# SamiPerttu/fundsp

Hardware: AMD Instinct MI355X
Metric: Msamples/s (whole node) for 65536-voice SVF+FM graph (higher is better)
Workload: dtype f32

## Files before the change

fundsp_amd/csrc/fd_device.hpp:

```cpp
#pragma once

#include "fd_nodes.hpp"
#include "fd_plan.hpp"
#include "fd_seq.hpp"

namespace fd {

constexpr int TILE_STRIDE = 68;

struct VLoad {
    const float* p;
    size_t stride;
    int slot;
    FD_D void f(float& x, FieldKind, const char*) { x = p[(size_t)slot++ * stride]; }
    FD_D void fi(float& x, FieldKind, const char*, int) { x = p[(size_t)slot++ * stride]; }
    FD_D void u32(uint32_t& x, FieldKind, const char*) { x = f2u(p[(size_t)slot++ * stride]); }
    FD_D void u64(uint64_t& x, FieldKind, const char*) {
        uint32_t lo = f2u(p[(size_t)slot * stride]);
        uint32_t hi = f2u(p[(size_t)(slot + 1) * stride]);
        slot += 2;
        x = ((uint64_t)hi << 32) | lo;
    }
    FD_D void enter(int) {}
    FD_D void leave() {}
// ... 2368 lines not shown
            }
        }
    }
    auto rounds_of = [&](auto* tag) {
        using GG = typename Pointee<decltype(tag)>::type;
        using T0 = Seg<GG, 0, 1>;
        using T1 = Seg<GG, 1, 2>;
        using T2 = Seg<GG, 2, 3>;
        GG& gg = reinterpret_cast<GG&>(g);
        auto loop = [&](auto&& block) {
            for (size_t it = 0; it < rounds; it++) {
                if (run && it >= (size_t)stage && it - stage < nblocks)
                    block(it - stage);
                __syncthreads();
            }
        };
        if (stage == 0) loop([&](size_t j) { ts_stage<T0, GG, true, W>(gg, R::cut[0][part], R::cut[0][part + 1], lane, nullptr, hand[grp][0][j & 1]); });
        else if (stage == 1) loop([&](size_t j) { ts_stage<T1, GG, false, W>(gg, R::cut[1][part], R::cut[1][part + 1], lane, hand[grp][0][j & 1], hand[grp][1][j & 1]); });
        else loop([&](size_t j) { pipe_stage<T2, GG, MODE_PROCESS, StageCfg<64, W, false, true, 64, OLM, FD_PIPE_PREFETCH != 0, MCM, (GPW == 2)>>(gg, 0, j * 64, 64, 64, T, V, lane, outw, nullptr, hand[grp][1][j & 1], nullptr, &mxl); });
    };
    using GL = typename LpOf<G>::type;
    bool lp = false;
    if constexpr (!SameType<GL, G>::v && FD_LP_ENABLE)
        lp = __builtin_amdgcn_ballot_w64(run && !lp_ok(g)) == 0ull && __builtin_amdgcn_ballot_w64(run) != 0ull;
    if (stage == 2) __builtin_amdgcn_s_setprio(1);
    if (lp) rounds_of((GL*)nullptr); else rounds_of((G*)nullptr);
    if (live && active && part == 0) {
        VStore<false> st{slots + v, stride, 0};
        VGate::W<VStore<false>> gate{&st, true};
        if (stage == 0) S0::visit(g, gate); else if (stage == 1) S1::visit(g, gate); else S2::visit(g, gate);
    }
}

template <class G, int GPW>
__global__ __launch_bounds__(64 * Ts3Roles<GPW>::WAVES) void k_render_ts3(float* __restrict__ slots, size_t stride, size_t V,
                                                                          float* __restrict__ out, size_t T, const void* aux) {
    if constexpr (TsPlan<G>::ok) render_ts3_body<G, GPW>(slots, stride, V, out, T, aux);
}
template <class G, int GPW, int MIX>
__global__ __launch_bounds__(64 * Ts3Roles<GPW>::WAVES) void k_render_ts3_mix(float* __restrict__ slots, size_t stride, size_t V,
                                                                              float* __restrict__ part, size_t T, const void* aux,
                                                                              const float* __restrict__ panw) {
    if constexpr (TsPlan<G>::ok) render_ts3_body<G, GPW, MIX>(slots, stride, V, part, T, aux, panw);
}

constexpr int PFS = 65;
template <class G>
struct PlanarPlan {
    static constexpr PipePlan P2 = pipe_plan<G>(2);
    static constexpr int N = Chain<G>::N;
    template <int S, int K1> struct Tiles {
        using S0 = Seg<G, 0, S == 1 ? N : K1>;
        using S1 = Seg<G, S == 1 ? 0 : K1, N>;
        static constexpr int W = S >= 2 ? S0::OUT : 0;
        static constexpr bool LATE_GIN = S >= 2 && S1::USES_GIN;
        static constexpr int D = G::IN > 0 ? (LATE_GIN ? S + 1 : 2) : 0;
        static constexpr int UNITS = G::IN * D + 2 * W * (S - 1) + 2 * G::OUT;
        static constexpr int SUB = UNITS <= 4 ? 32 : UNITS <= 9 ? 16 : UNITS <= 18 ? 8 : 0;
        static constexpr int WAVES = S + 1 + (G::IN > 0 ? 1 : 0);
        static constexpr bool ok = SUB >= 8 && WAVES <= 4 && G::OUT > 0;
    };
    static constexpr bool two_ok() {
        if constexpr (P2.S == 2) return Tiles<2, P2.K1>::ok; else return false;
    }
    static constexpr bool two = two_ok();
    static constexpr int S = two ? 2 : (Tiles<1, N>::ok ? 1 : 0);
    static constexpr int K1 = two ? P2.K1 : N;
    using T = Tiles<(S >= 1 ? S : 1), K1>;
};

template <class G, int MODE, int S, int K1, int GPW = 4>
FD_D void render_pipe_planar_body(float* __restrict__ slots, size_t stride, size_t V, const float* __restrict__ in,
                                  float* __restrict__ out, size_t T, size_t fstride, const void* aux, float* ring, uint32_t ring_cap) {
    using TL = typename PlanarPlan<G>::template Tiles<S, K1>;
    constexpr int NI = G::IN, NO = G::OUT;
    constexpr bool FEED = NI > 0;
// ... 154 lines not shown
        while (n > 0) { buf[k++] = (char)('0' + n % 10); n /= 10; }
        while (k > 0) put(buf[--k]);
    }
    FD_D void prefix() {
        for (int i = 0; i < depth; i++) { if (i) put('.'); putn(path[i]); }
        put(':');
    }
    FD_D void line(const char* name, int index, const char* suffix, int kind) {
        prefix();
        puts_(name);
        if (index >= 0) { put('['); putn(index); put(']'); }
        puts_(suffix);
        put(' ');
        putn(kind);
        put('\n');
    }
    FD_D void f(float&, FieldKind k, const char* name) { line(name, -1, "", (int)k); }
    FD_D void fi(float&, FieldKind k, const char* name, int index) { line(name, index, "", (int)k); }
    FD_D void u32(uint32_t&, FieldKind k, const char* name) { line(name, -1, "", (int)k); }
    FD_D void u64(uint64_t&, FieldKind k, const char* name) { line(name, -1, ".lo", (int)k); line(name, -1, ".hi", (int)k); }
    FD_D void enter(int i) { if (depth < 32) path[depth] = i; depth++; }
    FD_D void leave() { depth--; }
    bool keeps = false;
    FD_D void stale() { keeps = true; }
};
template <class G>
struct JitPipeSmall {
    static constexpr PipePlan P = pipe_plan<G>(0);
    static constexpr bool on = P.S >= 1 && Cost<G>::v >= 150;
    template <int GPW> static constexpr int threads() { return on ? 16 * GPW * PipeGeom<G::IN, (P.S >= 1 ? P.S : 1)>::WAVES : 64; }
};
template <class G, int GPW>
FD_D void jit_ts3_body(float* __restrict__ slots, size_t stride, size_t V, float* __restrict__ out, size_t T, const void* aux) {
    if constexpr (TsPlan<G>::ok) render_ts3_body<G, GPW>(slots, stride, V, out, T, aux);
}
template <class G, int GPW, int MIX>
FD_D void jit_ts3_mix_body(float* __restrict__ slots, size_t stride, size_t V, float* __restrict__ part, size_t T, const void* aux, const float* __restrict__ panw) {
    if constexpr (TsPlan<G>::ok && (MIX == MIX_SUM ? G::OUT <= 2 : G::OUT == 1)) render_ts3_body<G, GPW, MIX>(slots, stride, V, part, T, aux, panw);
}

template <class G, int MODE>
FD_D void jit_pipe_body(float* __restrict__ slots, size_t stride, size_t V, const float* __restrict__ in,
                        float* __restrict__ out, size_t T, const void* aux, float* ring, uint32_t ring_cap) {
    constexpr PipePlan P = pipe_plan<G>(0);
    if constexpr (P.S >= 1) render_pipe_body<G, MODE, P.S, P.K1, P.K2>(slots, stride, V, in, out, T, aux, ring, ring_cap);
}
template <class G, int MODE, int GPW>
FD_D void jit_pipe_small_body(float* __restrict__ slots, size_t stride, size_t V, const float* __restrict__ in,
                              float* __restrict__ out, size_t T, const void* aux, float* ring, uint32_t ring_cap) {
    constexpr PipePlan P = pipe_plan<G>(0);
    if constexpr (JitPipeSmall<G>::on) render_pipe_body<G, MODE, P.S, P.K1, P.K2, GPW>(slots, stride, V, in, out, T, aux, ring, ring_cap);
}
template <class G, int MODE, int MIX>
FD_D void jit_pipe_mix_body(float* __restrict__ slots, size_t stride, size_t V, const float* __restrict__ in,
                            float* __restrict__ part, size_t T, const void* aux, float* ring, uint32_t ring_cap, const float* __restrict__ panw) {
    constexpr PipePlan P = pipe_plan<G>(0);
    if constexpr (P.S >= 1 && (MIX == MIX_SUM || G::OUT == 1)) {
        if constexpr (MixGeom<(MIX == MIX_PAN ? 1 : G::OUT), 4, PipeTiles<G, P.S, P.K1, P.K2, 4>::SUB>::ok)
            render_pipe_body<G, MODE, P.S, P.K1, P.K2, 4, MIX>(slots, stride, V, in, part, T, aux, ring, ring_cap, panw);
    }
}
constexpr bool jit_mix_channels_ok(int channels) { return (31 * 1024) / 4 / (channels * MIX_ROW * 4) >= 8; }
static_assert(jit_mix_channels_ok(3) && !jit_mix_channels_ok(4) && MixGeom<3, 4, 64>::ok && !MixGeom<4, 4, 64>::ok, "fused mix-down: at most three output channels at four voice groups per workgroup");
template <class G, int MODE>
FD_D void jit_events_mix_body(float* __restrict__ slots, size_t stride, size_t V, const float* __restrict__ in, float* __restrict__ part, size_t T,
                              const double* __restrict__ ev, const int* __restrict__ fade, double time0, double sr, const void* aux, float* ring,
                              uint32_t ring_cap) {
    if constexpr (G::OUT <= 2) render_events_body<G, MODE, true>(slots, stride, V, in, part, T, ev, fade, time0, sr, aux, ring, ring_cap);
}
template <class G, int MODE>
FD_D void jit_score_mix_body(float* __restrict__ slots, size_t stride, size_t V, const float* __restrict__ in, float* __restrict__ part, size_t T,
// ... 10 lines not shown
FD_D void jit_pipe_planar_body(float* __restrict__ slots, size_t stride, size_t V, const float* __restrict__ in,
                               float* __restrict__ out, size_t T, size_t fstride, const void* aux, float* ring, uint32_t ring_cap) {
    using PP = PlanarPlan<G>;
    if constexpr (PP::S >= 1) render_pipe_planar_body<G, MODE, PP::S, PP::K1>(slots, stride, V, in, out, T, fstride, aux, ring, ring_cap);
}
template <class G>
struct JitPipePlanarThreads {
    static constexpr int v = PlanarPlan<G>::S >= 1 ? 256 * PlanarPlan<G>::T::WAVES : 64;
};
template <class G>
struct JitPipeThreads {
    static constexpr PipePlan P = pipe_plan<G>(0);
    static constexpr int v = P.S >= 1 ? 64 * PipeGeom<G::IN, (P.S >= 1 ? P.S : 1)>::WAVES : 64;
};

template <class G>
constexpr GraphTraits graph_traits(bool run_time) {
    constexpr PipePlan P = pipe_plan<G>(0);
    constexpr bool heavy = Cost<G>::v >= 150, ts = TsPlan<G>::ok;
    GraphTraits t{};
    t.nin = G::IN, t.nout = G::OUT, t.nrings = G::RINGS;
    t.wpb_planar = RenderGeom<G, LAYOUT_PLANAR>::WPB;
    for (int want = 0; want < 4; want++) t.pipe_stages[want] = !run_time ? pipe_plan<G>(want).S : (want == 1 && pipe_plan<G>(1).S < 1) ? 0 : P.S;
    t.pipe_min_t = PipeMinT<G>::v;
    t.pipe_threads = P.S >= 1 ? JitPipeThreads<G>::v : 0;
    t.pipe_planar_threads = PlanarPlan<G>::S >= 1 ? JitPipePlanarThreads<G>::v : 0;
    t.planar_stages = PlanarPlan<G>::S;
    t.wide_waves = run_time && WideChain<G>::on ? WideChain<G>::W : 0;
    t.heavy = heavy;
    t.small_groups_planar = t.small_groups_mix = heavy && !run_time;
    t.ts_ok = ts, t.ts_round2 = ts && !run_time, t.ts_mix_ok = ts && (!run_time || G::OUT <= 2);
    t.mix_sum_ok = !run_time || jit_mix_channels_ok(G::OUT);
    t.has_fast = !SameType<typename FastOf<G>::type, G>::v;
    return t;
}
template <class G>
FD_D void describe_body(char* out, int cap, GraphTraits* traits) {
    if (threadIdx.x != 0 || blockIdx.x != 0) return;
    G g;
    VDescribeDev d{out, 0, cap, {0}, 0};
    g.visit(d);
    out[d.pos] = 0;
    GraphTraits t = graph_traits<G>(true);
    t.note_fresh = G::RINGS == 0 && !d.keeps;
    *traits = t;
}

}
```

fundsp_amd/csrc/fd_engine.hpp:

```cpp
#pragma once

#include <functional>
#include <string>
#include <type_traits>
#include <vector>

#include "fd_device.hpp"
#include "fd_opts.hpp"

namespace fd {

struct SlotInfo {
    std::string name;
    int kind;
};

struct VDescribe {
    std::vector<SlotInfo>* out;
    std::vector<int> path;
    std::string prefix() const {
        std::string s;
        for (size_t i = 0; i < path.size(); i++) {
            if (i) s += ".";
            s += std::to_string(path[i]);
// ... 68 lines not shown
struct RenderArgs {
    float* slots; size_t stride, V; const float* in; float* out; size_t T, fstride; const void* aux; float* ring; uint32_t ring_cap;
    const float* panw;
    hipStream_t s;
};
template <int N> using IntC = std::integral_constant<int, N>;
template <class G, class F>
void with_gpw(int gpw, F&& f) {
    if constexpr (Cost<G>::v >= 150) {
        if (gpw == 1) return f(IntC<1>{});
        if (gpw == 2) return f(IntC<2>{});
    }
    f(IntC<4>{});
}
template <class G, int MODE, int WANT, int MIX = MIX_NONE>
void launch_pipe(const RenderPlan& p, const RenderArgs& a) {
    constexpr PipePlan P = pipe_plan<G>(WANT);
    if constexpr (P.S >= 1) {
        constexpr int WAVES = PipeGeom<G::IN, P.S>::WAVES;
        with_gpw<G>(p.gpw, [&](auto gpw) {
            constexpr int GPW = decltype(gpw)::value;
            if constexpr (MIX == MIX_NONE)
                hipLaunchKernelGGL((k_render_pipe<G, MODE, P.S, P.K1, P.K2, GPW>), dim3(p.grid), dim3(16 * GPW * WAVES), 0, a.s, a.slots, a.stride, a.V,
                                   a.in, a.out, a.T, a.aux, a.ring, a.ring_cap);
            else
                hipLaunchKernelGGL((k_render_pipe_mix<G, MODE, P.S, P.K1, P.K2, GPW, MIX>), dim3(p.grid), dim3(16 * GPW * WAVES), 0, a.s, a.slots,
                                   a.stride, a.V, a.in, a.out, a.T, a.aux, a.ring, a.ring_cap, a.panw);
        });
    }
}
template <class G, int MIX>
void launch_ts(const RenderPlan& p, const RenderArgs& a) {
    auto ts3 = [&](auto gpw) {
        constexpr int GPW = decltype(gpw)::value, THREADS = 64 * Ts3Roles<GPW>::WAVES;
        if constexpr (MIX != MIX_NONE)
            hipLaunchKernelGGL((k_render_ts3_mix<G, GPW, MIX>), dim3(p.grid), dim3(THREADS), 0, a.s, a.slots, a.stride, a.V, a.out, a.T, a.aux, a.panw);
        else
            hipLaunchKernelGGL((k_render_ts3<G, GPW>), dim3(p.grid), dim3(THREADS), 0, a.s, a.slots, a.stride, a.V, a.out, a.T, a.aux);
    };
    if constexpr (MIX == MIX_NONE)
        if (p.ts_round2) {
            if (p.ts_round2 == 2) hipLaunchKernelGGL((k_render_ts<G, 2, 2>), dim3(p.grid), dim3(64 * 5), 0, a.s, a.slots, a.stride, a.V, a.out, a.T, a.aux);
            else hipLaunchKernelGGL((k_render_ts<G, 2, 1>), dim3(p.grid), dim3(64 * 4), 0, a.s, a.slots, a.stride, a.V, a.out, a.T, a.aux);
            return;
        }
    if (p.gpw == 1) ts3(IntC<1>{});
    else ts3(IntC<2>{});
}
template <class G> struct TspKernel { static constexpr bool ok = false; };
template <class G> void launch_tsp(const RenderPlan& p, const RenderArgs& a);
template <class G, int MODE, int LAYOUT>
void launch_single(const RenderPlan& p, const RenderArgs& a) {
    constexpr int WPB = RenderGeom<G, LAYOUT>::WPB;
    const size_t fstride = LAYOUT == LAYOUT_VOICE_MINOR ? (size_t)p.vpw : a.fstride;
    hipLaunchKernelGGL((k_render<G, MODE, LAYOUT, WPB>), dim3(p.grid), dim3(64 * WPB), 0, a.s, a.slots, a.stride, a.V, a.in, a.out, a.T, fstride, a.aux,
                       a.ring, a.ring_cap);
}
template <class G, int MODE>
void launch_render_mode(const RenderPlan& p, const RenderArgs& a, int layout) {
    if (p.family == LK_PIPELINE_PLANAR) {
        using PP = PlanarPlan<G>;
        if constexpr (PP::S >= 1)
            with_gpw<G>(p.gpw, [&](auto gpw) {
                constexpr int GPW = decltype(gpw)::value;
                hipLaunchKernelGGL((k_render_pipe_planar<G, MODE, PP::S, PP::K1, GPW>), dim3(p.grid), dim3(64 * GPW * PP::T::WAVES), 0, a.s, a.slots,
                                   a.stride, a.V, a.in, a.out, a.T, a.fstride, a.aux, a.ring, a.ring_cap);
            });
// ... 179 lines not shown
```

fundsp_amd/csrc/fd_jit.hip:

```cpp
#ifndef _GNU_SOURCE
#define _GNU_SOURCE 1
#endif
#include <dlfcn.h>
#include <link.h>
#include <limits.h>
#include <stdlib.h>
#include <hip/hiprtc.h>

#include <cstring>
#include <fstream>
#include <map>
#include <memory>
#include <mutex>
#include <cstdio>
#include <sstream>

#include "fd_engine.hpp"
#include "fd_resynth.hpp"

namespace fd {

int jit_compile_src(const std::string& src, const std::string& type_expr, std::vector<char>* code, std::string* log);
std::string jit_source_mix(const std::string& type_expr, const std::string& prelude);
std::string jit_source_score(const std::string& type_expr, const std::string& prelude);
// ... 253 lines not shown
        std::string log;
        const std::string type = which ? "typename fd::FastOf<" + jm->type_expr + ">::type" : jm->type_expr;
        if (jit_compile_src(jit_source_mix(type, jm->prelude), jm->type_expr, &mm->code, &log) == 0) jm->mix[which] = mm;
        else {
            jm->mix_failed[which] = true;
            fprintf(stderr, "fundsp_hip: the mix-down / time-split kernels of this graph failed to compile: %s\n", log.c_str());
        }
    }
    return jm->mix[which].get();
}

void jit_render(JitModule* jm, float* slots, size_t stride, size_t V, const float* in, float* outp, size_t T, size_t fstride,
                int layout, int mode, const void* aux, float* ring, uint32_t ring_cap, hipStream_t s, JitModule* base, int which) {
    if (V == 0 || T == 0) return;
    const JitFuncs* f = jm->get();
    if (!f) return jit_launch_failed();
    GraphTraits traits = jm->traits;
    const size_t cus = (size_t)simd_count() / 4;
    const bool aligned = (((uintptr_t)in | (uintptr_t)outp) & 15) == 0;
    RenderPlan p = plan_render(traits, tl_opts, cus, V, T, layout, mode, fstride, aligned);
    const JitMix::Dev* tf = nullptr;
    if (p.family == LK_TIME_SPLIT) {
        JitMix* mm = jit_extra_module(base, which);
        tf = mm ? mm->get() : nullptr;
        if (!tf) {
            traits.ts_ok = false;
            p = plan_render(traits, tl_opts, cus, V, T, layout, mode, fstride, aligned);
        }
    }
    tl_opts.last_kernel = p.family;
    const unsigned gpw = (unsigned)p.gpw;
    if (p.family == LK_TIME_SPLIT) {
        void* targs[] = {&slots, &stride, &V, &outp, &T, &aux};
        hipModuleLaunchKernel(tf->ts[gpw - 1], p.grid, 1, 1, 64u * (gpw == 1 ? Ts3Roles<1>::WAVES : Ts3Roles<2>::WAVES), 1, 1, 0, s, targs, nullptr);
        return;
    }
    if (p.family == LK_PIPELINE) {
        void* pargs[] = {&slots, &stride, &V, &in, &outp, &T, &aux, &ring, &ring_cap};
        hipModuleLaunchKernel(gpw == 4 ? f->pipe[mode] : f->pipe_small[gpw - 1][mode], p.grid, 1, 1, (unsigned)traits.pipe_threads / 4 * gpw, 1, 1, 0, s, pargs,
                              nullptr);
        return;
    }
    if (p.family == LK_SINGLE_WAVE && layout == LAYOUT_VOICE_MINOR) fstride = (size_t)p.vpw;
    void* args[] = {&slots, &stride, &V, &in, &outp, &T, &fstride, &aux, &ring, &ring_cap};
    if (p.family == LK_WIDE_CHAIN)
        hipModuleLaunchKernel(f->wide[mode][layout], p.grid, 1, 1, 64u * (unsigned)traits.wide_waves, 1, 1, 0, s, args, nullptr);
    else if (p.family == LK_PIPELINE_PLANAR)
        hipModuleLaunchKernel(f->pipe_planar[mode], p.grid, 1, 1, (unsigned)traits.pipe_planar_threads, 1, 1, 0, s, args, nullptr);
    else
        hipModuleLaunchKernel(f->render[mode][layout], p.grid, 1, 1, 64 * gpw, 1, 1, 0, s, args, nullptr);
}

}

std::string jit_source(const std::string& type_expr, const std::string& prelude) {
    std::string s;
    s += "#include \"fd_device.hpp\"\n";
    if (!prelude.empty()) s += "namespace fd {\n" + prelude + "\n}\n";
    s += "namespace fd { using JitG = " + type_expr + "; }\n";
    s += "using fd::JitG;\n";
    s += "constexpr int JIT_WPB0 = fd::RenderGeom<JitG, 0>::WPB;\nconstexpr int JIT_WPB1 = fd::RenderGeom<JitG, 1>::WPB;\n";
    s += "extern \"C\" __global__ __launch_bounds__(64) void jit_lifecycle(float* slots, size_t stride, size_t first, "
         "size_t count, int op, double sr, const uint64_t* seeds, const void* aux, float* ring, uint32_t cap) {\n"
         "  fd::lifecycle_body<JitG>(slots, stride, first, count, op, sr, seeds, aux, ring, cap); }\n";
    for (int mode = 0; mode < 2; mode++)
        for (int layout = 0; layout < 2; layout++) {
            std::string m = std::to_string(mode), l = std::to_string(layout);
// ... 32 lines not shown
        s += "extern \"C\" __global__ __launch_bounds__(JIT_PIPE_PLANAR_THREADS) void jit_pipe_planar_" + m +
             "(float* __restrict__ slots, size_t stride, size_t V, const float* __restrict__ in, float* __restrict__ out, "
             "size_t T, size_t fstride, const void* aux, float* ring, uint32_t cap) {\n"
             "  fd::jit_pipe_planar_body<JitG, " + m + ">(slots, stride, V, in, out, T, fstride, aux, ring, cap); }\n";
    }
    for (int mode = 0; mode < 2; mode++) {
        std::string m = std::to_string(mode);
        s += "extern \"C\" __global__ __launch_bounds__(256) void jit_events_" + m +
             "(float* __restrict__ slots, size_t stride, size_t V, const float* __restrict__ in, float* __restrict__ out, "
             "size_t T, const double* __restrict__ ev, const int* __restrict__ fade, double time0, double sr, const void* aux, "
             "float* ring, uint32_t cap) {\n"
             "  fd::render_events_body<JitG, " + m + ">(slots, stride, V, in, out, T, ev, fade, time0, sr, aux, ring, cap); }\n";
    }
    s += "extern \"C\" __global__ void jit_describe(char* out, int cap, fd::GraphTraits* traits) { fd::describe_body<JitG>(out, cap, traits); }\n";
    return s;
}

std::string jit_source_mix(const std::string& type_expr, const std::string& prelude) {
    std::string s;
    s += "#include \"fd_device.hpp\"\n";
    if (!prelude.empty()) s += "namespace fd {\n" + prelude + "\n}\n";
    s += "namespace fd { using JitG = " + type_expr + "; }\nusing fd::JitG;\n";
    s += "constexpr int JIT_PIPE_THREADS = fd::JitPipeThreads<JitG>::v;\n";
    for (int mix = 1; mix <= 2; mix++)
        for (int mode = 0; mode < 2; mode++) {
            std::string m = std::to_string(mode), x = std::to_string(mix);
            s += "extern \"C\" __global__ __launch_bounds__(JIT_PIPE_THREADS) void jit_pipe_mix_" + x + "_" + m +
                 "(float* __restrict__ slots, size_t stride, size_t V, const float* __restrict__ in, float* __restrict__ part, "
                 "size_t T, const void* aux, float* ring, uint32_t cap, const float* __restrict__ panw) {\n"
                 "  fd::jit_pipe_mix_body<JitG, " + m + ", " + x + ">(slots, stride, V, in, part, T, aux, ring, cap, panw); }\n";
        }
    for (int g = 1; g <= 2; g++) {
        std::string gs = std::to_string(g);
        s += "extern \"C\" __global__ __launch_bounds__(64 * fd::Ts3Roles<" + gs + ">::WAVES) void jit_ts3_g" + gs +
             "(float* __restrict__ slots, size_t stride, size_t V, float* __restrict__ out, size_t T, const void* aux) {\n"
             "  fd::jit_ts3_body<JitG, " + gs + ">(slots, stride, V, out, T, aux); }\n";
        for (int mix = 1; mix <= 2; mix++) {
            std::string x = std::to_string(mix);
            s += "extern \"C\" __global__ __launch_bounds__(64 * fd::Ts3Roles<" + gs + ">::WAVES) void jit_ts3_mix_g" + gs + "_" + x +
                 "(float* __restrict__ slots, size_t stride, size_t V, float* __restrict__ part, size_t T, const void* aux, const float* __restrict__ panw) {\n"
                 "  fd::jit_ts3_mix_body<JitG, " + gs + ", " + x + ">(slots, stride, V, part, T, aux, panw); }\n";
        }
    }
    for (int mode = 0; mode < 2; mode++) {
        std::string m = std::to_string(mode);
        s += "extern \"C\" __global__ __launch_bounds__(256) void jit_events_mix_" + m +
             "(float* __restrict__ slots, size_t stride, size_t V, const float* __restrict__ in, float* __restrict__ part, "
             "size_t T, const double* __restrict__ ev, const int* __restrict__ fade, double time0, double sr, const void* aux, "
             "float* ring, uint32_t cap) {\n"
             "  fd::jit_events_mix_body<JitG, " + m + ">(slots, stride, V, in, part, T, ev, fade, time0, sr, aux, ring, cap); }\n";
    }
    return s;
}

std::string jit_source_score(const std::string& type_expr, const std::string& prelude) {
    std::string s;
    s += "#include \"fd_device.hpp\"\n";
    if (!prelude.empty()) s += "namespace fd {\n" + prelude + "\n}\n";
    s += "namespace fd { using JitG = " + type_expr + "; }\nusing fd::JitG;\n";
    for (int mode = 0; mode < 2; mode++) {
        std::string m = std::to_string(mode);
        s += "extern \"C\" __global__ __launch_bounds__(256) void jit_score_" + m +
             "(float* __restrict__ slots, size_t stride, size_t V, const float* __restrict__ in, float* __restrict__ out, "
             "size_t T, const fd::ScoreData sc, double time0, double sr, const void* aux, float* ring, uint32_t cap) {\n"
             "  fd::render_score_body<JitG, " + m + ">(slots, stride, V, in, out, T, sc, time0, sr, aux, ring, cap); }\n";
        s += "extern \"C\" __global__ __launch_bounds__(256) void jit_score_mix_" + m +
             "(float* __restrict__ slots, size_t stride, size_t V, const float* __restrict__ in, float* __restrict__ part, "
             "size_t T, const fd::ScoreData sc, double time0, double sr, const void* aux, float* ring, uint32_t cap) {\n"
             "  fd::jit_score_mix_body<JitG, " + m + ">(slots, stride, V, in, part, T, sc, time0, sr, aux, ring, cap); }\n";
        s += "extern \"C\" __global__ __launch_bounds__(256) void jit_score_notes_" + m +
             "(const float* __restrict__ slots, float* __restrict__ stage, int* __restrict__ flag, size_t stride, size_t V, "
             "const float* __restrict__ in, size_t in_T, float* __restrict__ out, size_t T, const fd::ScoreData sc, double time0, double sr, const void* aux) {\n"
// ... 184 lines not shown
            } else {
                jm->fast_failed = true;
                fprintf(stderr, "fundsp_hip: tolerance-mode variant failed to compile, rendering exactly: %s\n", log.c_str());
            }
        }
        return jm->fast.get();
    };
    if (traits.ts_ok || traits.has_fast)
        out->prepare_render = [jm, fast_module](size_t voices, bool fast) {
            JitModule* fm = (fast && jm->traits.has_fast) ? fast_module() : nullptr;
            if (fm) fm->get();
            if (wants_time_split_module(jm->traits, (size_t)simd_count() / 4, voices))
                if (JitMix* mm = jit_extra_module(jm.get(), fm ? 1 : 0)) mm->get();
        };
    if (traits.has_fast)
        out->render_fast = [jm, fast_module](float* slots, size_t stride, size_t V, const float* in, float* outp, size_t T, size_t fstride,
                                             int layout, int mode, const void* aux, float* ring, uint32_t ring_cap, hipStream_t s) {
            JitModule* fm = fast_module();
            jit_render(fm ? fm : jm.get(), slots, stride, V, in, outp, T, fstride, layout, mode, aux, ring, ring_cap, s, jm.get(), fm ? 1 : 0);
        };
    auto mix_module = [jm](int which) -> JitMix* { return jit_extra_module(jm.get(), which); };
    auto mix_launch = [jm, mix_module](int which, float* slots, size_t stride, size_t V, const float* in, float* part, size_t T, int mix, int mode,
                           const void* aux, float* ring, uint32_t ring_cap, const float* panw, hipStream_t s) -> bool {
        if (V == 0 || T == 0) return true;
        const RenderPlan p = plan_render_mix(jm->traits, tl_opts, (size_t)simd_count() / 4, V, T, mix, mode);
        if (p.family == LK_NONE) return false;
        JitMix* mm = mix_module(which);
        if (!mm) return false;
        const JitMix::Dev* f = mm->get();
        if (!f) { jit_launch_failed(); return true; }
        tl_opts.last_kernel = p.family;
        if (p.family == LK_TIME_SPLIT) {
            void* targs[] = {&slots, &stride, &V, &part, &T, &aux, &panw};
            hipModuleLaunchKernel(f->tsm[p.gpw - 1][mix - 1], p.grid, 1, 1, 64u * (p.gpw == 1 ? Ts3Roles<1>::WAVES : Ts3Roles<2>::WAVES), 1, 1, 0, s, targs, nullptr);
            return true;
        }
        void* pargs[] = {&slots, &stride, &V, &in, &part, &T, &aux, &ring, &ring_cap, &panw};
        hipModuleLaunchKernel(f->fn[mix - 1][mode], p.grid, 1, 1, (unsigned)jm->traits.pipe_threads, 1, 1, 0, s, pargs, nullptr);
        return true;
    };
    if (traits.pipe_stages[0] >= 1 && (traits.nout == 1 || traits.mix_sum_ok)) {
        out->prepare_mix = [mix_module](bool fast) {
            if (JitMix* mm = mix_module(fast ? 1 : 0)) mm->get();
        };
        out->render_mix = [mix_launch](float* slots, size_t stride, size_t V, const float* in, float* part, size_t T, int mix, int mode,
                                       const void* aux, float* ring, uint32_t ring_cap, const float* panw, hipStream_t s) {
            return mix_launch(0, slots, stride, V, in, part, T, mix, mode, aux, ring, ring_cap, panw, s);
        };
        if (traits.has_fast)
            out->render_mix_fast = [mix_launch](float* slots, size_t stride, size_t V, const float* in, float* part, size_t T, int mix, int mode,
                                                const void* aux, float* ring, uint32_t ring_cap, const float* panw, hipStream_t s) {
                return mix_launch(1, slots, stride, V, in, part, T, mix, mode, aux, ring, ring_cap, panw, s);
            };
    }
    if (traits.nout <= 2)
        out->render_events_mix = [mix_module](float* slots, size_t stride, size_t V, const float* in, float* part, size_t T, const double* ev,
                                              const int* fade, double time0, double sr, int mode, const void* aux, float* ring,
                                              uint32_t ring_cap, hipStream_t s) -> bool {
            if (V == 0 || T == 0) return true;
            JitMix* mm = mix_module(0);
            if (!mm) return false;
            const JitMix::Dev* f = mm->get();
            if (!f) { jit_launch_failed(); return true; }
            void* args[] = {&slots, &stride, &V, &in, &part, &T, &ev, &fade, &time0, &sr, &aux, &ring, &ring_cap};
            hipModuleLaunchKernel(f->ev[mode], (unsigned)(((V + 63) / 64 + 3) / 4), 1, 1, 256, 1, 1, 0, s, args, nullptr);
            tl_opts.last_kernel = LK_EVENTS;
            return true;
// ... 62 lines not shown
```

fundsp_amd/csrc/fd_nodes.hpp:

```cpp
#pragma once

#include "fd_math.hpp"

#define FD_D __device__ __forceinline__

namespace fd {

enum FieldKind { PARAM = 0, COEF = 1, STATE = 2 };

template <class V> FD_HD auto note_stale(V& v, int) -> decltype(v.stale(), void()) { v.stale(); }
template <class V> FD_HD void note_stale(V&, long) {}

constexpr int PH_SIMD = 0, PH_REM = 1, PH_TICK = 2;

struct Aux;
struct Ctx {
    const Aux* aux;
    float* ring;
    uint32_t ring_cap;
    size_t vstride;
    int next_ring;
    uint32_t* ring_need = nullptr;
    FD_HD float* claim_ring() { return ring + (size_t)(next_ring++) * ring_cap * vstride; }
    FD_HD void want_positions(uint32_t want) const {
// ... 183 lines not shown
    template <int PH> FD_HD void step(const float* in, float* out) {
        if (PH == PH_SIMD) {
            float tmp = phase;
            phase += in[0] * sample_duration;
            out[0] = wide_sinf(tmp * F32_TAU);
        } else {
            float p = phase;
            phase += in[0] * sample_duration;
            phase -= __builtin_floorf(phase);
            out[0] = sinf_musl(p * F32_TAU);
        }
    }
    template <int PH> FD_HD void step2(const v2f* in, v2f* out) {
        if (PH == PH_SIMD) {
            v2f d = in[0] * sample_duration;
            float t0 = phase;
            phase += d.x;
            float t1 = phase;
            phase += d.y;
            out[0] = wide_sin2(v2f{t0, t1} * F32_TAU, tmax);
        } else {
            float o0, o1, i0 = in[0].x, i1 = in[0].y;
            this->template step<PH>(&i0, &o0);
            this->template step<PH>(&i1, &o1);
            out[0] = v2f{o0, o1};
        }
    }
    template <int PH> FD_HD void skip(const float* in) { phase += in[0] * sample_duration; }
    template <int PH> FD_HD void skip2(const v2f* in) {
        v2f d = in[0] * sample_duration;
        phase += d.x;
        phase += d.y;
    }
};

constexpr float BOUND_MARGIN = 1.0000005f;
template <class T> struct OutBound {
    static constexpr bool has = false;
    static FD_HD float get(const T&) { return __builtin_inff(); }
};
template <> struct OutBound<Constant<1>> {
    static constexpr bool has = true;
    static FD_HD float get(const Constant<1>& c) { return __builtin_fabsf(c.value[0]); }
};
constexpr float SINE_OUT_BOUND = 16.0f;
template <> struct OutBound<Sine> {
    static constexpr bool has = true;
    static FD_HD float get(const Sine&) { return SINE_OUT_BOUND; }
};

struct SineB : Sine {
    static constexpr float TURNS_MAX = 2047.0f;
    FD_HD void begin_block(int) { tmax = __builtin_inff(); }
    FD_HD void begin_block(int size, float in_bound) {
        const float pmax = __builtin_fabsf(phase) + (float)size * (in_bound * __builtin_fabsf(sample_duration));
        tmax = (pmax < TURNS_MAX && f2u(phase) != 0x80000000u) ? 0.0f : __builtin_inff();
    }
    template <int PH> FD_HD void step2(const v2f* in, v2f* out) {
        if (PH == PH_SIMD) {
            v2f d = in[0] * sample_duration;
            float t0 = phase;
            phase += d.x;
            float t1 = phase;
            phase += d.y;
            out[0] = wide_sin2(v2f{t0, t1} * F32_TAU);
        } else {
            Sine::template step2<PH>(in, out);
        }
    }
};
template <> struct OutBound<SineB> {
    static constexpr bool has = true;
    static FD_HD float get(const SineB&) { return SINE_OUT_BOUND; }
};

struct SineFast : Sine {
    FD_HD void begin_block(int) {}
    FD_HD bool tripped() const { return false; }
    template <int PH> FD_HD void step(const float* in, float* out) {
        if (PH == PH_SIMD) {
            float tmp = phase;
            phase += in[0] * sample_duration;
            out[0] = fast_sin1(tmp * F32_TAU);
        } else {
            Sine::template step<PH>(in, out);
        }
    }
    template <int PH> FD_HD void step2(const v2f* in, v2f* out) {
        if (PH == PH_SIMD) {
            v2f d = in[0] * sample_duration;
            float t0 = phase;
            phase += d.x;
            float t1 = phase;
            phase += d.y;
            out[0] = v2f{fast_sin1(t0 * F32_TAU), fast_sin1(t1 * F32_TAU)};
        } else {
            Sine::template step2<PH>(in, out);
        }
    }
};

struct SinePlain : Sine {
    template <int PH> FD_HD void step2(const v2f* in, v2f* out) {
        if (PH == PH_SIMD) {
            v2f d = in[0] * sample_duration;
            float t0 = phase;
            phase += d.x;
            float t1 = phase;
            phase += d.y;
            out[0] = v2f{wide_sin1(t0 * F32_TAU, tmax), wide_sin1(t1 * F32_TAU, tmax)};
        } else {
            Sine::template step2<PH>(in, out);
        }
    }
};

template <int NIN>
struct Dsf {
    static constexpr int IN = NIN, OUT = 1, RINGS = 0;
    static constexpr uint64_t ID = 55;
    float phase, roughness, harmonic_spacing, sample_duration, has_phase, initial_phase;
    uint64_t hash;
    template <class V> FD_HD void visit(V& v) {
        v.f(phase, STATE, "phase");
        v.f(roughness, NIN > 1 ? STATE : PARAM, "roughness");
        v.f(harmonic_spacing, PARAM, "harmonic_spacing");
        v.f(sample_duration, COEF, "sample_duration");
        v.f(has_phase, PARAM, "has_initial_phase");
        v.f(initial_phase, PARAM, "initial_phase");
        v.u64(hash, STATE, "hash");
    }
    FD_HD void bind(Ctx&) {}
// ... 3614 lines not shown
```

fundsp_amd/csrc/fd_plan.hpp:

```cpp
#pragma once

#ifndef __HIPCC_RTC__
#include <stddef.h>
#endif

#include "fd_opts.hpp"

namespace fd {

constexpr int LAYOUT_VOICE_MINOR = 0, LAYOUT_PLANAR = 1;
constexpr int MODE_PROCESS = 0, MODE_TICK = 1;
constexpr int MIX_NONE = 0, MIX_SUM = 1, MIX_PAN = 2;

#ifndef FD_TS_MIN_T
#define FD_TS_MIN_T 64
#endif
#ifndef FD_PLANAR_PIPE_MIN_T
#define FD_PLANAR_PIPE_MIN_T 16
#endif

struct GraphTraits {
    int nin, nout, nrings;
    int wpb_planar;
    int pipe_stages[4];
    int pipe_min_t;
    int pipe_threads;
    int pipe_planar_threads;
    int planar_stages;
    int wide_waves;
    bool heavy;
    bool small_groups_planar;
    bool small_groups_mix;
    bool ts_ok;
    bool ts_round2;
    bool ts_mix_ok;
    bool mix_sum_ok;
    bool has_fast;
    bool note_fresh;
    bool tsp_ok;
};

struct RenderPlan {
    int family;
    int gpw;
    unsigned grid;
    int vpw;
    int want;
    int ts_round2;
};

inline int voices_per_wave(size_t V, int simds) {
    int vpw = 64;
    while (vpw > 16 && (V + vpw - 1) / vpw < (size_t)simds) vpw >>= 1;
    return vpw;
}

constexpr int pipe_want(int pipe_split) { return pipe_split == 4 ? 1 : pipe_split == 2 ? 2 : pipe_split == 3 ? 3 : 0; }

inline unsigned plan_grid(size_t groups, int gpw) { return (unsigned)((groups + gpw - 1) / gpw); }

inline int pipe_gpw(bool small_groups, size_t groups, size_t cus) { return small_groups && groups <= cus ? 1 : small_groups && groups <= 2 * cus ? 2 : 4; }

inline bool plan_time_split(const LaunchOpts& o, size_t cus, size_t groups, size_t T, int mode) {
    return o.pipe_split == 1 && mode == MODE_PROCESS && T % 64 == 0 && T >= FD_TS_MIN_T && groups <= 2 * cus;
}

inline bool wants_time_split_module(const GraphTraits& g, size_t cus, size_t voices) { return g.ts_ok && (voices + 63) / 64 <= 2 * cus; }

inline RenderPlan plan_render(const GraphTraits& g, const LaunchOpts& o, size_t cus, size_t V, size_t T, int layout, int mode, size_t fstride,
                              bool io_aligned16) {
    const size_t groups = (V + 63) / 64;
    const bool voice_minor = layout == LAYOUT_VOICE_MINOR;
// ... 39 lines not shown
```

Measured before the change: 667,600.

## Split sine carrier into phase and eval roles in time-split pipeline

Adds a six-wave time-split kernel body for graphs whose middle stage is a sine carrier and GPW is 2. One wave per group runs the modulator plus the phase accumulation, a separate wave evaluates the sine from the handed-off phase arguments, and a third runs the downstream filter stage, all linked through double-buffered LDS handoffs. The intent is to move the serial phase recurrence off the path of the costly sine evaluation so the three stages overlap. In exchange there is an extra pipeline round, more LDS and more waves per block, and priority is raised on the eval wave by default.

```diff
diff --git a/fundsp_amd/csrc/fd_device.hpp b/fundsp_amd/csrc/fd_device.hpp
--- a/fundsp_amd/csrc/fd_device.hpp
+++ b/fundsp_amd/csrc/fd_device.hpp
@@ -2424,16 +2424,180 @@
     }
 }
 
+template <class T> struct IsSineSeam { static constexpr bool v = false; };
+template <> struct IsSineSeam<Sine> { static constexpr bool v = true; };
+template <> struct IsSineSeam<SineFast> { static constexpr bool v = true; };
+template <bool C, class A, class B> struct PickType { using type = A; };
+template <class A, class B> struct PickType<false, A, B> { using type = B; };
+template <class G, int A, bool HEAD = true> struct StageNode {
+    struct None {};
+    static constexpr bool LEAF = A == 0 && Chain<G, HEAD>::N == 1;
+    using type = typename PickType<LEAF, G, None>::type;
+    static FD_D G& get(G& g) { return g; }
+};
+template <class X, class Y, int A, bool HEAD> struct StageNode<Pipe<X, Y>, A, HEAD> {
+    static constexpr int NX = Chain<X, HEAD>::N;
+    static constexpr bool INX = A < NX;
+    using SX = StageNode<X, INX ? A : 0, HEAD>;
+    using SY = StageNode<Y, INX ? 0 : A - NX, false>;
+    using type = typename PickType<INX, typename SX::type, typename SY::type>::type;
+    static FD_D auto& get(Pipe<X, Y>& g) { if constexpr (INX) return SX::get(g.x); else return SY::get(g.y); }
+};
+template <class G, bool TS = TsPlan<G>::ok> struct TsSeam { static constexpr bool on = false; };
+template <class G> struct TsSeam<G, true> { static constexpr bool on = IsSineSeam<typename StageNode<G, 1>::type>::v; };
+static_assert(TsSeam<Pipe<Pipe<Unop<Pipe<Constant<1>, Sine>, UAddScalar>, Sine>, FixedSvf>>::on && TsSeam<Pipe<Pipe<Constant<1>, SineFast>, FixedSvf>>::on &&
+              !TsSeam<Pipe<Noise, Biquad>>::on, "the three-role body: sine carriers yes, config 2's noise | ff | fb no");
+#ifndef FD_TS2_ROLES
+#define FD_TS2_ROLES 1
+#endif
+#ifndef FD_TS2_PRIO
+#define FD_TS2_PRIO 2
+#endif
+template <class G, int GPW> struct Ts3Geom {
+    static constexpr bool SEAM = FD_TS2_ROLES != 0 && GPW == 2 && TsSeam<G>::on;
+    static constexpr int WAVES = SEAM ? 6 : Ts3Roles<GPW>::WAVES;
+};
+
+template <class T0, class SN, class GG>
+FD_D void ts_front(GG& g, int lane, v2f (*hout)[32][64]) {
+    static_assert(T0::IN == 0 && T0::OUT == 1, "a mono generator stage in front of the carrier");
+    auto& car = SN::get(g);
+    T0::begin(g, 64);
+    const GG snap = g;
+    for (int i8 = 0; i8 < 64; i8 += 8) {
+#pragma unroll
+        for (int k = 0; k < 4; k++) {
+            v2f pi[1], po[1], pa[1];
+            T0::template step2<PH_SIMD>(g, pi, pi, po);
+            car.template front2<PH_SIMD>(po, pa);
+            hout[0][(i8 >> 1) + k][lane] = pa[0];
+        }
+    }
+    if (__builtin_expect(T0::tripped(g), 0)) {
+        g = snap;
+        for (int i = 0; i < 64; i++) {
+            float fi[1], fo[1], fa[1];
+            T0::template step<PH_SIMD>(g, fi, fi, fo);
+            car.template front<PH_SIMD>(fo, fa);
+            reinterpret_cast<float*>(&hout[0][i >> 1][lane])[i & 1] = fa[0];
+        }
+    }
+    T0::end(g);
+    car.end_simd();
+}
+template <class SN, class GG>
+FD_D void ts_eval(GG& g, int lane, v2f (*hin)[32][64], v2f (*hout)[32][64]) {
+    auto& car = SN::get(g);
+    v2f ahead[4];
+#pragma unroll
+    for (int k = 0; k < 4; k++) ahead[k] = hin[0][k][lane];
+    car.back_begin(ahead[0].x);
+    for (int i8 = 0; i8 < 64; i8 += 8) {
+        const int nx = i8 + 8 < 64 ? i8 + 8 : i8;
+#pragma unroll
+        for (int k = 0; k < 4; k++) {
+            v2f pa[1], po[1];
+            pa[0] = ahead[k];
+            ahead[k] = hin[0][(nx >> 1) + k][lane];
+            car.back2(pa, po);
+            hout[0][(i8 >> 1) + k][lane] = po[0];
+        }
+    }
+    if (__builtin_expect(car.tripped(), 0)) {
+        for (int i = 0; i < 64; i++) {
+            float fa[1], fo[1];
+            fa[0] = reinterpret_cast<const float*>(&hin[0][i >> 1][lane])[i & 1];
+            car.back(fa, fo);
+            reinterpret_cast<float*>(&hout[0][i >> 1][lane])[i & 1] = fo[0];
+        }
+    }
+}
+
+template <class G, int MIX = MIX_NONE>
+FD_D void render_ts3_seam_body(float* __restrict__ slots, size_t stride, size_t V, float* __restrict__ out, size_t T, const void* aux, const float* __restrict__ panw = nullptr) {
+    constexpr int GPW = 2, W = 1;
+    using S01 = Seg<G, 0, 2>;
+    using S2 = Seg<G, 2, 3>;
+    static_assert(Seg<G, 0, 1>::OUT == 1 && Seg<G, 1, 2>::OUT == 1, "one channel per cut");
+    __shared__ v2f hand[GPW][2][2][W][32][64];
+    const int lane = threadIdx.x & 63, w = __builtin_amdgcn_readfirstlane(threadIdx.x >> 6);
+    const int grp = w & 1, role = w < 2 ? 2 : (w < 4 ? 0 : 1);
+    const size_t v0 = ((size_t)blockIdx.x * GPW + grp) * 64, v = v0 + lane;
+    const bool live = v0 < stride, active = v < V;
+    const size_t nblocks = T / 64, rounds = nblocks + 2;
+    constexpr int NM = MIX == MIX_PAN ? 2 : G::OUT;
+    constexpr int NTC = MIX == MIX_PAN ? 1 : G::OUT;
+    using MG = MixGeom<NTC, GPW, 64>;
+    constexpr bool WLDS = MIX == MIX_PAN;
+    constexpr int OLM = MIX == MIX_NONE ? 0 : (MIX == MIX_PAN ? 4 : 2), MCM = MIX == MIX_NONE ? 0 : MG::MC;
+    static_assert(MIX == MIX_NONE || MG::ok, "mix tile does not fit");
+    float* outw = MIX == MIX_NONE ? out + v0 : out + (v0 / 64) * (size_t)NM * T;
+    __shared__ __attribute__((aligned(16))) float mixt[MIX == MIX_NONE ? 1 : GPW][MIX == MIX_NONE ? 4 : MG::FLOATS];
+    __shared__ __attribute__((aligned(16))) v2f mixw[WLDS ? GPW : 1][WLDS ? 64 : 1];
+    MixLane mxl{&mixt[MIX == MIX_NONE ? 0 : grp][0], active ? lane : 64, {}, nullptr};
+    const bool run = live && (MIX != MIX_NONE || active);
+    G g{};
+    Ctx ctx{static_cast<const Aux*>(aux), nullptr, 0, stride, 0};
+    g.bind(ctx);
+    if (live && role != 1) {
+        VLoad ld{slots + v, stride, 0};
+        VGate::W<VLoad> gate{&ld, true};
+        if (role == 0) S01::visit(g, gate); else S2::visit(g, gate);
+    }
+    if constexpr (MIX != MIX_NONE) {
+        if (role == 2) {
+            if (!active) {
+#pragma unroll 1
+                for (int r = 0; r < NTC * MCM; r++) mxl.tile[r * MIX_ROW + lane] = 0.0f;
+            }
+            if constexpr (MIX == MIX_PAN) {
+                if (live) mixw[grp][lane] = v2f{panw[v0 + lane], panw[stride + v0 + lane]};
+                mxl.wlds = &mixw[grp][0];
+            }
+        }
+    }
+    auto rounds_of = [&](auto* tag) {
+        using GG = typename Pointee<decltype(tag)>::type;
+        using T0 = Seg<GG, 0, 1>;
+        using SN = StageNode<GG, 1>;
+        using T2 = Seg<GG, 2, 3>;
+        GG& gg = reinterpret_cast<GG&>(g);
+        auto loop = [&](auto&& block) {
+            for (size_t it = 0; it < rounds; it++) {
+                if (run && it >= (size_t)role && it - role < nblocks)
+                    block(it - role);
+                __syncthreads();
+            }
+        };
+        if (role == 0) loop([&](size_t j) { ts_front<T0, SN, GG>(gg, lane, hand[grp][0][j & 1]); });
+        else if (role == 1) loop([&](size_t j) { ts_eval<SN, GG>(gg, lane, hand[grp][0][j & 1], hand[grp][1][j & 1]); });
+        else loop([&](size_t j) { pipe_stage<T2, GG, MODE_PROCESS, StageCfg<64, W, false, true, 64, OLM, FD_PIPE_PREFETCH != 0, MCM, true>>(gg, 0, j * 64, 64, 64, T, V, lane, outw, nullptr, hand[grp][1][j & 1], nullptr, &mxl); });
+    };
+    using GL = typename LpOf<G>::type;
+    bool lp = false;
+    if constexpr (!SameType<GL, G>::v && FD_LP_ENABLE)
+        lp = __builtin_amdgcn_ballot_w64(run && !lp_ok(g)) == 0ull && __builtin_amdgcn_ballot_w64(run) != 0ull;
+    if (FD_TS2_PRIO != 0 && role == (FD_TS2_PRIO == 2 ? 1 : 2)) __builtin_amdgcn_s_setprio(1);
+    if (lp) rounds_of((GL*)nullptr); else rounds_of((G*)nullptr);
+    if (live && active && role != 1) {
+        VStore<false> st{slots + v, stride, 0};
+        VGate::W<VStore<false>> gate{&st, true};
+        if (role == 0) S01::visit(g, gate); else S2::visit(g, gate);
+    }
+}
+
 template <class G, int GPW>
-__global__ __launch_bounds__(64 * Ts3Roles<GPW>::WAVES) void k_render_ts3(float* __restrict__ slots, size_t stride, size_t V,
-                                                                          float* __restrict__ out, size_t T, const void* aux) {
-    if constexpr (TsPlan<G>::ok) render_ts3_body<G, GPW>(slots, stride, V, out, T, aux);
+__global__ __launch_bounds__((64 * Ts3Geom<G, GPW>::WAVES)) void k_render_ts3(float* __restrict__ slots, size_t stride, size_t V,
+                                                                            float* __restrict__ out, size_t T, const void* aux) {
+    if constexpr (Ts3Geom<G, GPW>::SEAM) render_ts3_seam_body<G>(slots, stride, V, out, T, aux);
+    else if constexpr (TsPlan<G>::ok) render_ts3_body<G, GPW>(slots, stride, V, out, T, aux);
 }
 template <class G, int GPW, int MIX>
-__global__ __launch_bounds__(64 * Ts3Roles<GPW>::WAVES) void k_render_ts3_mix(float* __restrict__ slots, size_t stride, size_t V,
-                                                                              float* __restrict__ part, size_t T, const void* aux,
-                                                                              const float* __restrict__ panw) {
-    if constexpr (TsPlan<G>::ok) render_ts3_body<G, GPW, MIX>(slots, stride, V, part, T, aux, panw);
+__global__ __launch_bounds__((64 * Ts3Geom<G, GPW>::WAVES)) void k_render_ts3_mix(float* __restrict__ slots, size_t stride, size_t V,
+                                                                                float* __restrict__ part, size_t T, const void* aux,
+                                                                                const float* __restrict__ panw) {
+    if constexpr (Ts3Geom<G, GPW>::SEAM) render_ts3_seam_body<G, MIX>(slots, stride, V, part, T, aux, panw);
+    else if constexpr (TsPlan<G>::ok) render_ts3_body<G, GPW, MIX>(slots, stride, V, part, T, aux, panw);
 }
 
 constexpr int PFS = 65;
@@ -2654,11 +2818,15 @@
 };
 template <class G, int GPW>
 FD_D void jit_ts3_body(float* __restrict__ slots, size_t stride, size_t V, float* __restrict__ out, size_t T, const void* aux) {
-    if constexpr (TsPlan<G>::ok) render_ts3_body<G, GPW>(slots, stride, V, out, T, aux);
+    if constexpr (Ts3Geom<G, GPW>::SEAM) render_ts3_seam_body<G>(slots, stride, V, out, T, aux);
+    else if constexpr (TsPlan<G>::ok) render_ts3_body<G, GPW>(slots, stride, V, out, T, aux);
 }
 template <class G, int GPW, int MIX>
 FD_D void jit_ts3_mix_body(float* __restrict__ slots, size_t stride, size_t V, float* __restrict__ part, size_t T, const void* aux, const float* __restrict__ panw) {
-    if constexpr (TsPlan<G>::ok && (MIX == MIX_SUM ? G::OUT <= 2 : G::OUT == 1)) render_ts3_body<G, GPW, MIX>(slots, stride, V, part, T, aux, panw);
+    if constexpr (TsPlan<G>::ok && (MIX == MIX_SUM ? G::OUT <= 2 : G::OUT == 1)) {
+        if constexpr (Ts3Geom<G, GPW>::SEAM) render_ts3_seam_body<G, MIX>(slots, stride, V, part, T, aux, panw);
+        else render_ts3_body<G, GPW, MIX>(slots, stride, V, part, T, aux, panw);
+    }
 }
 
 template <class G, int MODE>
@@ -2735,6 +2903,7 @@
     t.ts_ok = ts, t.ts_round2 = ts && !run_time, t.ts_mix_ok = ts && (!run_time || G::OUT <= 2);
     t.mix_sum_ok = !run_time || jit_mix_channels_ok(G::OUT);
     t.has_fast = !SameType<typename FastOf<G>::type, G>::v;
+    t.ts_threads[0] = 64 * Ts3Geom<G, 1>::WAVES, t.ts_threads[1] = 64 * Ts3Geom<G, 2>::WAVES;
     return t;
 }
 template <class G>
diff --git a/fundsp_amd/csrc/fd_engine.hpp b/fundsp_amd/csrc/fd_engine.hpp
--- a/fundsp_amd/csrc/fd_engine.hpp
+++ b/fundsp_amd/csrc/fd_engine.hpp
@@ -124,7 +124,7 @@
 template <class G, int MIX>
 void launch_ts(const RenderPlan& p, const RenderArgs& a) {
     auto ts3 = [&](auto gpw) {
-        constexpr int GPW = decltype(gpw)::value, THREADS = 64 * Ts3Roles<GPW>::WAVES;
+        constexpr int GPW = decltype(gpw)::value, THREADS = 64 * Ts3Geom<G, GPW>::WAVES;
         if constexpr (MIX != MIX_NONE)
             hipLaunchKernelGGL((k_render_ts3_mix<G, GPW, MIX>), dim3(p.grid), dim3(THREADS), 0, a.s, a.slots, a.stride, a.V, a.out, a.T, a.aux, a.panw);
         else
diff --git a/fundsp_amd/csrc/fd_jit.hip b/fundsp_amd/csrc/fd_jit.hip
--- a/fundsp_amd/csrc/fd_jit.hip
+++ b/fundsp_amd/csrc/fd_jit.hip
@@ -309,7 +309,7 @@
     const unsigned gpw = (unsigned)p.gpw;
     if (p.family == LK_TIME_SPLIT) {
         void* targs[] = {&slots, &stride, &V, &outp, &T, &aux};
-        hipModuleLaunchKernel(tf->ts[gpw - 1], p.grid, 1, 1, 64u * (gpw == 1 ? Ts3Roles<1>::WAVES : Ts3Roles<2>::WAVES), 1, 1, 0, s, targs, nullptr);
+        hipModuleLaunchKernel(tf->ts[gpw - 1], p.grid, 1, 1, (unsigned)traits.ts_threads[gpw - 1], 1, 1, 0, s, targs, nullptr);
         return;
     }
     if (p.family == LK_PIPELINE) {
@@ -408,12 +408,12 @@
         }
     for (int g = 1; g <= 2; g++) {
         std::string gs = std::to_string(g);
-        s += "extern \"C\" __global__ __launch_bounds__(64 * fd::Ts3Roles<" + gs + ">::WAVES) void jit_ts3_g" + gs +
+        s += "extern \"C\" __global__ __launch_bounds__((64 * fd::Ts3Geom<JitG, " + gs + ">::WAVES)) void jit_ts3_g" + gs +
              "(float* __restrict__ slots, size_t stride, size_t V, float* __restrict__ out, size_t T, const void* aux) {\n"
              "  fd::jit_ts3_body<JitG, " + gs + ">(slots, stride, V, out, T, aux); }\n";
         for (int mix = 1; mix <= 2; mix++) {
             std::string x = std::to_string(mix);
-            s += "extern \"C\" __global__ __launch_bounds__(64 * fd::Ts3Roles<" + gs + ">::WAVES) void jit_ts3_mix_g" + gs + "_" + x +
+            s += "extern \"C\" __global__ __launch_bounds__((64 * fd::Ts3Geom<JitG, " + gs + ">::WAVES)) void jit_ts3_mix_g" + gs + "_" + x +
                  "(float* __restrict__ slots, size_t stride, size_t V, float* __restrict__ part, size_t T, const void* aux, const float* __restrict__ panw) {\n"
                  "  fd::jit_ts3_mix_body<JitG, " + gs + ", " + x + ">(slots, stride, V, part, T, aux, panw); }\n";
         }
@@ -664,7 +664,7 @@
         tl_opts.last_kernel = p.family;
         if (p.family == LK_TIME_SPLIT) {
             void* targs[] = {&slots, &stride, &V, &part, &T, &aux, &panw};
-            hipModuleLaunchKernel(f->tsm[p.gpw - 1][mix - 1], p.grid, 1, 1, 64u * (p.gpw == 1 ? Ts3Roles<1>::WAVES : Ts3Roles<2>::WAVES), 1, 1, 0, s, targs, nullptr);
+            hipModuleLaunchKernel(f->tsm[p.gpw - 1][mix - 1], p.grid, 1, 1, (unsigned)jm->traits.ts_threads[p.gpw - 1], 1, 1, 0, s, targs, nullptr);
             return true;
         }
         void* pargs[] = {&slots, &stride, &V, &in, &part, &T, &aux, &ring, &ring_cap, &panw};
diff --git a/fundsp_amd/csrc/fd_nodes.hpp b/fundsp_amd/csrc/fd_nodes.hpp
--- a/fundsp_amd/csrc/fd_nodes.hpp
+++ b/fundsp_amd/csrc/fd_nodes.hpp
@@ -239,6 +239,22 @@
         phase += d.x;
         phase += d.y;
     }
+    template <int PH> FD_HD void front2(const v2f* in, v2f* arg) {
+        v2f d = in[0] * sample_duration;
+        float t0 = phase;
+        phase += d.x;
+        float t1 = phase;
+        phase += d.y;
+        arg[0] = v2f{t0, t1} * F32_TAU;
+    }
+    template <int PH> FD_HD void front(const float* in, float* arg) {
+        float tmp = phase;
+        phase += in[0] * sample_duration;
+        arg[0] = tmp * F32_TAU;
+    }
+    FD_HD void back_begin(float arg0) { tmax = f2u(arg0) == 0x80000000u ? __builtin_inff() : 0.0f; }
+    FD_HD void back2(const v2f* arg, v2f* out) { out[0] = wide_sin2(arg[0], tmax); }
+    FD_HD void back(const float* arg, float* out) { out[0] = wide_sinf(arg[0]); }
 };
 
 constexpr float BOUND_MARGIN = 1.0000005f;
@@ -305,6 +321,9 @@
             Sine::template step2<PH>(in, out);
         }
     }
+    FD_HD void back_begin(float) {}
+    FD_HD void back2(const v2f* arg, v2f* out) { out[0] = fast_sin2(arg[0]); }
+    FD_HD void back(const float* arg, float* out) { out[0] = fast_sin1(arg[0]); }
 };
 
 struct SinePlain : Sine {
diff --git a/fundsp_amd/csrc/fd_plan.hpp b/fundsp_amd/csrc/fd_plan.hpp
--- a/fundsp_amd/csrc/fd_plan.hpp
+++ b/fundsp_amd/csrc/fd_plan.hpp
@@ -38,6 +38,7 @@
     bool has_fast;
     bool note_fresh;
     bool tsp_ok;
+    int ts_threads[2];
 };
 
 struct RenderPlan {
```

Result: no change. 668,100 (median of 2 runs) (+0.1%).
